# Ascend-Research/HeadPoseEstimation-WHENet

Hardware: NVIDIA H100
Metric: head-crops/sec @224x224 bf16 (higher is better)
Workload: dtype bf16

## Files before the change

headposeestimation-whenet_b200/csrc/kernels_fused.cuh:

```cuda
#pragma once
#include <algorithm>

#include "kernels_tc.cuh"

namespace whenet {
namespace fused {

using tc::BK;
using tc::BM;

constexpr size_t K1_MAX_SMEM = 227 * 1024 - 256;
constexpr float kDwScale = 4.0f;

struct K1Params {
    const void* in;
    const void* wt_aug;
    const float* w_dw;
    const void* w_dw16;
    const float* b_dw;
    void* out;
    float* partial;
    const float *w_se1t, *b_se1, *w_se2, *b_se2;
    float* gate;
    int* se_counter;
// ... 15 lines not shown
    int nkb;
    int pitchE;
    int PY;
    int spr_log2;
    int smem_A, smem_W, smem_C, smem_E;
    int* tflag;
    int chunks_per_cta;
};

__device__ __forceinline__ void cp_async16(uint32_t dst, const void* src, bool valid) {
    const uint32_t sz = valid ? 16u : 0u;
    asm volatile("cp.async.cg.shared.global [%0], [%1], 16, %2;" ::"r"(dst), "l"(src), "r"(sz) : "memory");
}
__device__ __forceinline__ void sts128(uint32_t addr, const uint4& v) {
    asm volatile("st.shared.v4.b32 [%0], {%1,%2,%3,%4};" ::"r"(addr), "r"(v.x), "r"(v.y), "r"(v.z), "r"(v.w) : "memory");
}
__device__ __forceinline__ void lds64(uint32_t addr, uint32_t& a, uint32_t& b) {
    asm volatile("ld.shared.v2.b32 {%0,%1}, [%2];" : "=r"(a), "=r"(b) : "r"(addr));
}
__device__ __forceinline__ float4 lds_f4(uint32_t addr) {
    float4 v;
    asm volatile("ld.shared.v4.f32 {%0,%1,%2,%3}, [%4];" : "=f"(v.x), "=f"(v.y), "=f"(v.z), "=f"(v.w) : "r"(addr));
    return v;
}
__device__ __forceinline__ void ffma2(float2& d, const float2& a, const float2& b) {
    d.x = fmaf(a.x, b.x, d.x);
    d.y = fmaf(a.y, b.y, d.y);
}
template <typename T> __device__ __forceinline__ void unpack2(uint32_t u, float& lo, float& hi);
template <> __device__ __forceinline__ void unpack2<__nv_bfloat16>(uint32_t u, float& lo, float& hi) {
    lo = __uint_as_float(u << 16);
    hi = __uint_as_float(u & 0xffff0000u);
}
template <> __device__ __forceinline__ void unpack2<__half>(uint32_t u, float& lo, float& hi) {
    const float2 f = __half22float2(*reinterpret_cast<const __half2*>(&u));
    lo = f.x; hi = f.y;
}
template <typename T> __device__ __forceinline__ uint32_t pack2(float lo, float hi);
template <> __device__ __forceinline__ uint32_t pack2<__nv_bfloat16>(float lo, float hi) {
    const __nv_bfloat162 h = __floats2bfloat162_rn(lo, hi);
    return *reinterpret_cast<const uint32_t*>(&h);
}
template <> __device__ __forceinline__ uint32_t pack2<__half>(float lo, float hi) {
    const __half2 h = __floats2half2_rn(lo, hi);
    return *reinterpret_cast<const uint32_t*>(&h);
}
template <typename T> __device__ __forceinline__ uint32_t ones2();
template <> __device__ __forceinline__ uint32_t ones2<__nv_bfloat16>() { return 0x3f803f80u; }
template <> __device__ __forceinline__ uint32_t ones2<__half>() { return 0x3c003c00u; }

__device__ __forceinline__ uint32_t sw128(int r, int c) {
    return (uint32_t)((r >> 3) * 1024 + (r & 7) * 128 + ((c ^ (r & 7)) << 4));
}

__device__ __forceinline__ int div_small(int x, float inv) { return __float2int_rz(((float)x + 0.5f) * inv); }

template <int NP>
__device__ __forceinline__ void expand_row_to_e(const float (&d)[8 * NP], int nch16, int hr, uint32_t er, int cq) {
#pragma unroll
    for (int jj = 0; jj < NP; ++jj) {
        if (jj < nch16) {
#pragma unroll
            for (int i = 0; i < 2; ++i) {
                const uint32_t v = pack2<__half>(swish_from_half(d[8 * jj + 4 * i + 2 * hr]), swish_from_half(d[8 * jj + 4 * i + 2 * hr + 1]));
                asm volatile("st.shared.b32 [%0], %1;" ::"r"(er + (uint32_t)(16 * jj + 8 * i + cq) * 2u), "r"(v) : "memory");
            }
        }
    }
}

template <int KS, int S, int R>
__device__ __forceinline__ void dw_strip_hfma2(uint32_t erow, uint32_t e_rowstride, uint32_t pitchE, uint32_t wts, uint32_t w_pitch,
                                               const float4& bq, float2 (&acc)[R][2]) {
    constexpr int NCOL = (R - 1) * S + KS;
    __half2 hacc[R][2];
#pragma unroll
    for (int r = 0; r < R; ++r) { hacc[r][0] = __float2half2_rn(0.f); hacc[r][1] = __float2half2_rn(0.f); }
#pragma unroll
    for (int ky = 0; ky < KS; ++ky) {
        __half2 wr[KS][2];
#pragma unroll
        for (int kx = 0; kx < KS; ++kx) {
            uint32_t w0, w1;
            lds64(wts + (uint32_t)(ky * KS + kx) * w_pitch, w0, w1);
            wr[kx][0] = *reinterpret_cast<__half2*>(&w0); wr[kx][1] = *reinterpret_cast<__half2*>(&w1);
        }
        uint32_t ea = erow;
#pragma unroll
        for (int col = 0; col < NCOL; ++col) {
            uint32_t a, b;
            lds64(ea, a, b);
            ea += pitchE;
            const __half2 x01 = *reinterpret_cast<__half2*>(&a), x23 = *reinterpret_cast<__half2*>(&b);
#pragma unroll
            for (int r = 0; r < R; ++r) {
                const int kx = col - r * S;
                if (kx >= 0 && kx < KS) {
                    hacc[r][0] = __hfma2(x01, wr[kx][0], hacc[r][0]);
                    hacc[r][1] = __hfma2(x23, wr[kx][1], hacc[r][1]);
                }
            }
        }
        erow += e_rowstride;
    }
    const float2 sc = make_float2(kDwScale, kDwScale);
#pragma unroll
// ... 480 lines not shown
```

headposeestimation-whenet_b200/csrc/kernels_k1x.cuh:

```cuda
#pragma once
#include "kernels_dwse.cuh"

namespace whenet {
namespace fused {

template <int KS, int S, int HIN, int TH, int R, int CC, int CIN>
struct K1X {
    static constexpr int NT = 256;
    static constexpr int HO = (HIN + S - 1) / S;
    static constexpr int PAD = ((HO - 1) * S + KS - HIN > 0 ? (HO - 1) * S + KS - HIN : 0) / 2;
    static constexpr int TILES_X = HO / TH, TILES = TILES_X * TILES_X;
    static constexpr int IW = (TH - 1) * S + KS;
    static constexpr int NPIX = IW * IW;
    static constexpr int HALVES = (NPIX + 63) / 64;
    static constexpr int KCH = CIN / 8;
    static constexpr int KSTEPS = ((KCH + 2) & ~1) >> 1;
    static constexpr int SPR = (TH + R - 1) / R;
    static constexpr int NSTRIPS = TH * SPR;
    static constexpr int CV = CC / 4;
    static constexpr int PY = NT / CV;
    static constexpr uint32_t PITCHE = CC * 2 + 16;
    static constexpr int E_ROWS = NPIX + R * S + 16;
    static_assert(HO % TH == 0 && CIN % 8 == 0 && KCH + 1 < 8 && CC % 16 == 0 && CC <= 128, "tile plan");
    static constexpr uint32_t A_BYTES = (NPIX + 7) / 8 * 8 * 128;
    static constexpr uint32_t A_TX = NPIX * 128;
    static constexpr uint32_t W_BYTES = CC * 128;
    static constexpr uint32_t E_BYTES = (E_ROWS * PITCHE + 127) / 128 * 128;
    static constexpr uint32_t DWW_BYTES = KS * KS * CC * 2;
    static constexpr uint32_t CST_TX = DWW_BYTES + CC * 4;
    static constexpr uint32_t CST_BYTES = (CST_TX + 127) / 128 * 128;
    static constexpr uint32_t RED_BYTES = PY * CC * 4;
    static constexpr uint32_t OFF_W = A_BYTES, OFF_E = OFF_W + 2 * W_BYTES, OFF_C = OFF_E + E_BYTES, OFF_R = OFF_C + 2 * CST_BYTES;
    static constexpr size_t SMEM = (size_t)OFF_R + 2 * RED_BYTES + 1024;
    static_assert((A_BYTES | W_BYTES) % 1024 == 0 && DWW_BYTES % 16 == 0, "operand alignment");
    static_assert((size_t)HALVES * 64 * 128 + 1024 <= SMEM, "the last half's MMA stays inside the CTA's window");
    static_assert(2 * (SMEM + 1024 + 64) <= 228 * 1024, "two CTAs per SM");
};

template <int KS, int S, int HIN, int TH, int R, int CC, int CIN>
__global__ void __launch_bounds__(256, 2) k1x_kernel(const __grid_constant__ DwSeParams p) {
    using X = K1X<KS, S, HIN, TH, R, CC, CIN>;
    using T = __nv_bfloat16;
    extern __shared__ uint8_t smem_k1x[];
    __shared__ __align__(8) uint64_t bars[5];
    __shared__ int s_abort_mem;
    volatile int* s_abort = &s_abort_mem;
    const uint32_t s0 = (tc::smem_u32(smem_k1x) + 1023u) & ~1023u;
    const uint32_t sA = s0, sW = s0 + X::OFF_W, sE = s0 + X::OFF_E, sC = s0 + X::OFF_C, sR = s0 + X::OFF_R;
    const uint32_t b_a = tc::smem_u32(&bars[0]), b_w = b_a + 8, b_c = b_a + 24;

    const int tid = threadIdx.x, warp = tid >> 5, lane = tid & 31;
    const int wg = tid >> 7, wq = warp & 3;
    const int tile = blockIdx.x, n = blockIdx.y;
    const int tyi = tile / X::TILES_X;
    const int ty0 = tyi * TH, tx0 = (tile - tyi * X::TILES_X) * TH;
    const int iy0 = ty0 * S - X::PAD, ix0 = tx0 * S - X::PAD;
    const int C = p.C, n_chunks = p.n_chunks;

    if (tid == 0) {
        for (int i = 0; i < 5; ++i) tc::mbar_init(&bars[i], 1);
        s_abort_mem = 0;
        asm volatile("fence.mbarrier_init.release.cluster;" ::: "memory");
        asm volatile("prefetch.tensormap [%0];" ::"l"(&p.tmX) : "memory");
        asm volatile("prefetch.tensormap [%0];" ::"l"(&p.tmWx) : "memory");
        asm volatile("prefetch.tensormap [%0];" ::"l"(&p.tmW) : "memory");
    }
    __syncthreads();

    auto issue_w = [&](int j) {
        const uint32_t bar = b_w + 8 * (j & 1);
        tc::mbar::arrive_expect_tx(bar, X::W_BYTES);
        tc::mbar::tma_2d(sW + (j & 1) * X::W_BYTES, &p.tmWx, 0, j * CC, bar);
    };
    auto issue_c = [&](int j) {
        const uint32_t bar = b_c + 8 * (j & 1), dst = sC + (j & 1) * X::CST_BYTES;
        tc::mbar::arrive_expect_tx(bar, X::CST_TX);
        tc::mbar::tma_2d(dst, &p.tmW, j * CC, 0, bar);
        asm volatile("cp.async.bulk.shared::cluster.global.mbarrier::complete_tx::bytes [%0], [%1], %2, [%3];"
                     ::"r"(dst + X::DWW_BYTES), "l"(p.b_dw + j * CC), "r"((uint32_t)(CC * 4)), "r"(bar) : "memory");
    };
    if (tid == 0) {
        tc::mbar::arrive_expect_tx(b_a, X::A_TX);
        tc::mbar::tma_4d(sA, &p.tmX, 0, ix0, iy0, n, b_a);
        issue_w(0); issue_c(0);
        if (n_chunks > 1) { issue_w(1); issue_c(1); }
    }

    const int py = tid / X::CV, cv = tid - py * X::CV;
    const bool dw_active = py < X::PY;
    T* const out_t = reinterpret_cast<T*>(p.out) + (((long long)n * X::HO + ty0) * X::HO + tx0) * C + cv * 4;

    tc::mbar::wait(b_a, 0, s_abort, p.tflag);
    for (int r = tid; r < X::NPIX; r += X::NT) {
        const int ty = r / X::IW, tx = r - ty * X::IW;
        const int iy = iy0 + ty, ix = ix0 + tx;
        if (iy >= 0 && iy < HIN && ix >= 0 && ix < HIN) sts128(sA + sw128(r, X::KCH), make_uint4(ones2<T>(), 0u, 0u, 0u));
    }
    asm volatile("fence.proxy.async.shared::cta;" ::: "memory");
    __syncthreads();

    for (int j = 0; j < n_chunks; ++j) {
        const int buf = j & 1;
        const uint32_t par = (uint32_t)(j >> 1) & 1u;
        tc::mbar::wait(b_w + 8 * buf, par, s_abort, p.tflag);
        for (int u = wg; u < X::HALVES; u += 2) {
            float d[CC / 2];
            tc::wg_mma_m64<true, CC>(d, sA + (uint32_t)u * 64 * 128, X::A_BYTES, sW + buf * X::W_BYTES, X::W_BYTES, X::KSTEPS);
            tc::wg_wait<0>();
            const int r_lo = u * 64 + 16 * wq + (lane >> 2), cq = 2 * (lane & 3);
#pragma unroll
            for (int hr = 0; hr < 2; ++hr) {
                const int r = r_lo + 8 * hr;
                if (r < X::NPIX) expand_row_to_e<CC / 16>(d, CC / 16, hr, sE + (uint32_t)r * X::PITCHE, cq);
            }
        }
        __syncthreads();
        if (tid == 0 && j + 2 < n_chunks) issue_w(j + 2);

        tc::mbar::wait(b_c + 8 * buf, par, s_abort, p.tflag);
        if (dw_active && !*s_abort) {
            const uint32_t cst = sC + buf * X::CST_BYTES;
            const float4 bq = lds_f4(cst + X::DWW_BYTES + (uint32_t)cv * 16);
            float sum[4] = {0.f, 0.f, 0.f, 0.f};
            for (int sidx = py; sidx < X::NSTRIPS; sidx += X::PY) {
                const int oyl = sidx / X::SPR, oxl0 = (sidx - oyl * X::SPR) * R;
                float2 acc[R][2];
                dw_strip_hfma2<KS, S, R>(sE + (uint32_t)((oyl * S * X::IW + oxl0 * S) * X::PITCHE + cv * 8), X::IW * X::PITCHE, X::PITCHE,
                                         cst + (uint32_t)cv * 8, CC * 2, bq, acc);
                dw_strip_finish<T, R>(acc, TH - oxl0, out_t + ((long long)oyl * X::HO + oxl0) * C + j * CC, C, sum);
            }
            asm volatile("st.shared.v4.f32 [%0], {%1,%2,%3,%4};" ::"r"(sR + (uint32_t)(buf * X::RED_BYTES + (py * CC + cv * 4) * 4)),
                         "f"(sum[0]), "f"(sum[1]), "f"(sum[2]), "f"(sum[3]) : "memory");
        }
        __syncthreads();
        if (warp == X::NT / 32 - 1) {
            squeeze_sums<X::PY, CC>(sR + buf * X::RED_BYTES, p.partial + ((long long)n * X::TILES + tile) * C + j * CC, nullptr, 0.f, lane);
            if (lane == 0 && j + 2 < n_chunks) issue_c(j + 2);
        }
    }
}

#define WHENET_K1X_INSTANCES(F) F(3, 2, 112, 8, 4, 48, 16) F(3, 1, 56, 14, 7, 48, 24) F(5, 2, 56, 7, 4, 48, 24) F(3, 2, 28, 7, 7, 80, 40)

inline bool k1x_has_instance(int k, int s, int hin, int cin, int pad, const K1Params& pl, int R) {
#define K1X_MATCH(KS_, S_, HIN_, TH_, R_, CC_, CIN_)                                                                        \
    if (k == KS_ && s == S_ && hin == HIN_ && cin == CIN_ && pl.TH == TH_ && pl.TW == TH_ && R == R_ && pl.CC == CC_ && pl.NB == 1 && \
        pad == K1X<KS_, S_, HIN_, TH_, R_, CC_, CIN_>::PAD)                                                                  \
        return true;
    WHENET_K1X_INSTANCES(K1X_MATCH)
#undef K1X_MATCH
    return false;
}

template <typename T>
int launch_k1x(cudaStream_t stream, DwSeParams p, int k, int s, int hin, int cin, int th, int r, int cc, int n_crops) {
    static_assert(std::is_same<T, __nv_bfloat16>::value, "K1X runs the bf16 wgmma and the HFMA2 depthwise");
    p.N = n_crops;
    p.n_chunks = p.C / cc;
    p.chunks_per_cta = p.n_chunks;
#define K1X_GO(KS, S, HIN, TH, RR, CC, CIN)                                                                                  \
    if (k == KS && s == S && hin == HIN && cin == CIN && th == TH && r == RR && cc == CC) {                                  \
        using X = K1X<KS, S, HIN, TH, RR, CC, CIN>;                                                                          \
        auto kfn = k1x_kernel<KS, S, HIN, TH, RR, CC, CIN>;                                                                  \
        if (cudaFuncSetAttribute(kfn, cudaFuncAttributeMaxDynamicSharedMemorySize, (int)X::SMEM) != cudaSuccess) return -1;  \
        kfn<<<dim3(X::TILES, n_crops), X::NT, X::SMEM, stream>>>(p);                                                         \
        return 0;                                                                                                            \
    }
    WHENET_K1X_INSTANCES(K1X_GO)
#undef K1X_GO
    return 1;
}

}
}
```

headposeestimation-whenet_b200/csrc/kernels_tc.cuh:

```cuda
#pragma once
#include <cuda.h>
#include <cuda_bf16.h>
#include <cuda_fp16.h>
#include <cuda_runtime.h>
#include <stdint.h>

#include "kernels_simt.cuh"

namespace whenet {
namespace tc {


constexpr int BM = 128;
constexpr int BK = 64;
constexpr int A_STAGE_BYTES = BM * BK * 2;
constexpr int kAccPitch = 132;
__host__ __device__ constexpr uint32_t acc_tile_bytes(int cols) { return (uint32_t)cols * kAccPitch * 4u; }

__device__ __forceinline__ uint32_t smem_u32(const void* p) { return (uint32_t)__cvta_generic_to_shared(p); }

__device__ __forceinline__ void mbar_init(uint64_t* bar, uint32_t count) {
    asm volatile("mbarrier.init.shared::cta.b64 [%0], %1;" ::"r"(smem_u32(bar)), "r"(count) : "memory");
}
__device__ __forceinline__ bool mbar_wait(uint64_t* bar, uint32_t parity, int* tflag) {
// ... 13 lines not shown

namespace mbar {

__device__ __forceinline__ void wait(uint32_t bar_addr, uint32_t parity, volatile int* abort_flag, int* tflag) {
    for (uint32_t outer = 0; outer < (1u << 18); ++outer) {
        uint32_t done;
        asm volatile(
            "{\n\t.reg .pred p;\n\t.reg .u32 n;\n\t"
            "mov.u32 n, 64;\n"
            "MBAR_POLL_%=:\n\t"
            "mbarrier.try_wait.parity.shared::cta.b64 p, [%1], %2;\n\t"
            "@p bra MBAR_DONE_%=;\n\t"
            "sub.u32 n, n, 1;\n\t"
            "setp.ne.u32 p, n, 0;\n\t"
            "@p bra MBAR_POLL_%=;\n\t"
            "setp.eq.u32 p, n, 1;\n"
            "MBAR_DONE_%=:\n\t"
            "selp.u32 %0, 1, 0, p;\n\t}"
            : "=r"(done) : "r"(bar_addr), "r"(parity) : "memory");
        if (done) return;
        if (*abort_flag) return;
    }
    *abort_flag = 1;
    *reinterpret_cast<volatile int*>(tflag) = 1;
}
__device__ __forceinline__ void arrive(uint32_t bar_addr) {
    asm volatile("mbarrier.arrive.shared::cta.b64 _, [%0];" ::"r"(bar_addr) : "memory");
}
__device__ __forceinline__ void arrive_warp(uint32_t bar_addr) {
    __syncwarp();
    if ((threadIdx.x & 31) == 0) arrive(bar_addr);
}
__device__ __forceinline__ void arrive_expect_tx(uint32_t bar_addr, uint32_t bytes) {
    asm volatile("mbarrier.arrive.expect_tx.shared::cta.b64 _, [%0], %1;" ::"r"(bar_addr), "r"(bytes) : "memory");
}
__device__ __forceinline__ void tma_4d(uint32_t dst, const CUtensorMap* tm, int c0, int c1, int c2, int c3, uint32_t bar_addr) {
    asm volatile("cp.async.bulk.tensor.4d.shared::cluster.global.mbarrier::complete_tx::bytes [%0], [%1, {%2, %3, %4, %5}], [%6];"
                 ::"r"(dst), "l"(tm), "r"(c0), "r"(c1), "r"(c2), "r"(c3), "r"(bar_addr) : "memory");
}
__device__ __forceinline__ void tma_2d(uint32_t dst, const CUtensorMap* tm, int c0, int c1, uint32_t bar_addr) {
    asm volatile("cp.async.bulk.tensor.2d.shared::cluster.global.mbarrier::complete_tx::bytes [%0], [%1, {%2, %3}], [%4];"
                 ::"r"(dst), "l"(tm), "r"(c0), "r"(c1), "r"(bar_addr) : "memory");
}

}

__device__ __forceinline__ uint64_t make_desc(uint32_t saddr) {
    uint64_t d = 0;
    d |= (uint64_t)((saddr >> 4) & 0x3FFF);
    d |= (uint64_t)1 << 16;
    d |= (uint64_t)64 << 32;
    d |= (uint64_t)1 << 62;
    return d;
}

__device__ __forceinline__ void wg_fence() { asm volatile("wgmma.fence.sync.aligned;" ::: "memory"); }
__device__ __forceinline__ void wg_commit() { asm volatile("wgmma.commit_group.sync.aligned;" ::: "memory"); }
template <int N> __device__ __forceinline__ void wg_wait() { asm volatile("wgmma.wait_group.sync.aligned %0;" ::"n"(N) : "memory"); }

#define WG_D8(g) "+f"(d[8 * g]), "+f"(d[8 * g + 1]), "+f"(d[8 * g + 2]), "+f"(d[8 * g + 3]), \
                 "+f"(d[8 * g + 4]), "+f"(d[8 * g + 5]), "+f"(d[8 * g + 6]), "+f"(d[8 * g + 7])
#define WG_OPS_1 WG_D8(0)
#define WG_OPS_2 WG_OPS_1, WG_D8(1)
#define WG_OPS_3 WG_OPS_2, WG_D8(2)
#define WG_OPS_4 WG_OPS_3, WG_D8(3)
#define WG_OPS_5 WG_OPS_4, WG_D8(4)
#define WG_OPS_6 WG_OPS_5, WG_D8(5)
#define WG_OPS_7 WG_OPS_6, WG_D8(6)
#define WG_OPS_8 WG_OPS_7, WG_D8(7)
#define WG_REGS_1 "%0,%1,%2,%3,%4,%5,%6,%7"
#define WG_REGS_2 WG_REGS_1 ",%8,%9,%10,%11,%12,%13,%14,%15"
#define WG_REGS_3 WG_REGS_2 ",%16,%17,%18,%19,%20,%21,%22,%23"
#define WG_REGS_4 WG_REGS_3 ",%24,%25,%26,%27,%28,%29,%30,%31"
#define WG_REGS_5 WG_REGS_4 ",%32,%33,%34,%35,%36,%37,%38,%39"
#define WG_REGS_6 WG_REGS_5 ",%40,%41,%42,%43,%44,%45,%46,%47"
#define WG_REGS_7 WG_REGS_6 ",%48,%49,%50,%51,%52,%53,%54,%55"
#define WG_REGS_8 WG_REGS_7 ",%56,%57,%58,%59,%60,%61,%62,%63"
#define WG_TAIL_1 "16", "%8, %9", "%10"
#define WG_TAIL_2 "32", "%16, %17", "%18"
#define WG_TAIL_3 "48", "%24, %25", "%26"
#define WG_TAIL_4 "64", "%32, %33", "%34"
#define WG_TAIL_5 "80", "%40, %41", "%42"
#define WG_TAIL_6 "96", "%48, %49", "%50"
#define WG_TAIL_7 "112", "%56, %57", "%58"
#define WG_TAIL_8 "128", "%64, %65", "%66"
#define WG_ASM_(TY, REGS, NS, AB, SC, ...)                                                                              \
    asm volatile("{\n\t.reg .pred p;\n\tsetp.ne.b32 p, " SC ", 0;\n\t"                                                    \
                 "wgmma.mma_async.sync.aligned.m64n" NS "k16.f32." TY "." TY " {" REGS "}, " AB ", p, 1, 1, 0, 0;\n\t}" \
                 : __VA_ARGS__ : "l"(ad), "l"(bd), "r"(accumulate))
#define WG_ASM(TY, REGS, TAIL, OPS) WG_ASM_(TY, REGS, TAIL, OPS)
#define WG_CASE(k)                                                                                                 \
    if constexpr (N == 16 * k) {                                                                                   \
        if constexpr (BF16) WG_ASM("bf16", WG_REGS_##k, WG_TAIL_##k, WG_OPS_##k);                                  \
        else WG_ASM("f16", WG_REGS_##k, WG_TAIL_##k, WG_OPS_##k);                                                  \
    }

template <bool BF16, int N>
__device__ __forceinline__ void wgmma(float (&d)[N / 2], uint64_t ad, uint64_t bd, uint32_t accumulate) {
    static_assert(N % 16 == 0 && N >= 16 && N <= 128, "wgmma: N = 16, 32, ..., 128");
    WG_CASE(1) WG_CASE(2) WG_CASE(3) WG_CASE(4) WG_CASE(5) WG_CASE(6) WG_CASE(7) WG_CASE(8)
}
#undef WG_CASE
#undef WG_ASM
#undef WG_ASM_

template <int N> struct WgAcc { float d[2][N / 2]; };
// ... 574 lines not shown
```

headposeestimation-whenet_b200/csrc/whenet_api.cu:

```cuda
#include <cuda_bf16.h>
#include <cuda_fp16.h>
#include <cuda_runtime.h>

#include <algorithm>
#include <atomic>
#include <cmath>
#include <cstdarg>
#include <cstdio>
#include <cstdlib>
#include <cstring>
#include <map>
#include <string>
#include <thread>
#include <type_traits>
#include <vector>

#include "../../include/whenet_b200.h"
#include "api_error.h"
#include "kernels_simt.cuh"
#include "kernels_tc.cuh"
#include "kernels_fused.cuh"
#include "kernels_crop.cuh"
#include "kernels_overlay.cuh"
#include "kernels_k2.cuh"
// ... 266 lines not shown
        if (*p) cudaFree(*p);
        *p = nullptr;
    }
    for (float** p : {&c->d_partial, &c->d_gate, &c->d_pooled}) {
        if (*p) cudaFree(*p);
        *p = nullptr;
    }
    if (c->d_se_counter) cudaFree(c->d_se_counter);
    c->d_se_counter = nullptr;
    c->ws_chunk = 0;
}

int ensure_ws(whenet_ctx* c) {
    if (c->ws_chunk == c->chunk && c->bufA) return 0;
    free_ws(c);
    const size_t es = esize(c->precision), ch = (size_t)c->chunk;
    size_t io = 112ull * 112 * 32, ex = 49ull * 1280, dw = 0, part = 0;
    for (const BlockCfg& b : c->blocks) {
        io = std::max(io, (size_t)b.hout * b.hout * b.cout);
        if (b.has_expand) ex = std::max(ex, (size_t)b.hin * b.hin * b.cexp);
        dw = std::max(dw, (size_t)b.hout * b.hout * b.cexp);
        part = std::max(part, (size_t)((b.hout + 7) / 8) * b.cexp);
    }
    for (const K1Plan& pl : c->k1)
        if (pl.valid) part = std::max(part, (size_t)pl.p.tiles_x * pl.p.tiles_y * pl.p.Cexp);
    const BlockCfg& b1 = c->blocks[0];
    if (c->precision == WHENET_PRECISION_BF16) part = std::max(part, (size_t)(b1.hin / 14) * (b1.hin / 14) * b1.cexp);
    if (c->dw1.valid) part = std::max(part, (size_t)c->dw1.p.tiles_x * c->dw1.p.tiles_y * c->dw1.p.Cexp);
    c->ws_io = io; c->ws_ex = ex; c->ws_dw = dw; c->ws_part = part;
    CK(cudaMalloc(&c->bufA, ch * io * es));
    CK(cudaMalloc(&c->bufB, ch * io * es));
    CK(cudaMalloc(&c->bufE, ch * ex * es));
    CK(cudaMalloc(&c->bufD, ch * dw * es));
    CK(cudaMalloc(&c->d_partial, ch * part * sizeof(float)));
    CK(cudaMalloc(&c->d_gate, ch * 1152 * sizeof(float)));
    CK(cudaMalloc(&c->d_pooled, ch * 1280 * sizeof(float)));
    CK(cudaMalloc(&c->d_se_counter, ch * sizeof(int)));
    CK(cudaMemset(c->d_se_counter, 0, ch * sizeof(int)));
    for (int i = 0; i < 2; ++i) CK(cudaMalloc(&c->d_in[i], ch * kImgElems * sizeof(float)));
    c->ws_chunk = c->chunk;
    return 0;
}

PFN_cuTensorMapEncodeTiled_v12000 tmap_encode_fn() {
    static PFN_cuTensorMapEncodeTiled_v12000 fn = nullptr;
    if (!fn) {
        void* f = nullptr;
        cudaDriverEntryPointQueryResult q;
        if (cudaGetDriverEntryPoint("cuTensorMapEncodeTiled", &f, cudaEnableDefault, &q) == cudaSuccess && q == cudaDriverEntryPointSuccess)
            fn = reinterpret_cast<PFN_cuTensorMapEncodeTiled_v12000>(f);
    }
    return fn;
}
int make_tmap_w(CUtensorMap* tm, const void* base, int rows, int K, int box_rows, bool is_bf16) {
    auto fn = tmap_encode_fn();
    if (!fn) return fail(WHENET_ECUDA, "cuTensorMapEncodeTiled is not available from this driver");
    const cuuint64_t dims[2] = {(cuuint64_t)K, (cuuint64_t)rows};
    const cuuint64_t strides[1] = {(cuuint64_t)K * 2};
    const cuuint32_t box[2] = {64, (cuuint32_t)box_rows};
    const cuuint32_t estr[2] = {1, 1};
    const CUresult r = fn(tm, is_bf16 ? CU_TENSOR_MAP_DATA_TYPE_BFLOAT16 : CU_TENSOR_MAP_DATA_TYPE_FLOAT16, 2, const_cast<void*>(base), dims, strides,
                          box, estr, CU_TENSOR_MAP_INTERLEAVE_NONE, CU_TENSOR_MAP_SWIZZLE_128B, CU_TENSOR_MAP_L2_PROMOTION_L2_256B,
                          CU_TENSOR_MAP_FLOAT_OOB_FILL_NONE);
    if (r != CUDA_SUCCESS) return fail(WHENET_ECUDA, "cuTensorMapEncodeTiled(weights %dx%d, box %d) failed: %d", rows, K, box_rows, (int)r);
    return 0;
}

int make_tmap_kd_e(CUtensorMap* tm, const void* base, int n, int H, int C, int cc, int pw) {
    auto fn = tmap_encode_fn();
    if (!fn) return fail(WHENET_ECUDA, "cuTensorMapEncodeTiled is not available from this driver");
    const cuuint64_t dims[4] = {(cuuint64_t)C, (cuuint64_t)H, (cuuint64_t)H, (cuuint64_t)n};
    const cuuint64_t strides[3] = {(cuuint64_t)C * 2, (cuuint64_t)H * C * 2, (cuuint64_t)H * H * C * 2};
    const cuuint32_t box[4] = {(cuuint32_t)cc, (cuuint32_t)pw, (cuuint32_t)pw, 1};
    const cuuint32_t estr[4] = {1, 1, 1, 1};
    const CUresult r = fn(tm, CU_TENSOR_MAP_DATA_TYPE_FLOAT16, 4, const_cast<void*>(base), dims, strides, box, estr, CU_TENSOR_MAP_INTERLEAVE_NONE,
                          CU_TENSOR_MAP_SWIZZLE_NONE, CU_TENSOR_MAP_L2_PROMOTION_L2_128B, CU_TENSOR_MAP_FLOAT_OOB_FILL_NONE);
    if (r != CUDA_SUCCESS) return fail(WHENET_ECUDA, "cuTensorMapEncodeTiled(KD tile %dx%dx%dx%d, box %dx%dx%d) failed: %d", n, H, H, C, pw, pw, cc, (int)r);
    return 0;
}
int make_tmap_k1x_in(CUtensorMap* tm, const void* base, int n, int H, int C, int iw) {
    auto fn = tmap_encode_fn();
    if (!fn) return fail(WHENET_ECUDA, "cuTensorMapEncodeTiled is not available from this driver");
    const cuuint64_t dims[4] = {(cuuint64_t)C, (cuuint64_t)H, (cuuint64_t)H, (cuuint64_t)n};
    const cuuint64_t strides[3] = {(cuuint64_t)C * 2, (cuuint64_t)H * C * 2, (cuuint64_t)H * H * C * 2};
    const cuuint32_t box[4] = {64, (cuuint32_t)iw, (cuuint32_t)iw, 1};
    const cuuint32_t estr[4] = {1, 1, 1, 1};
    const CUresult r = fn(tm, CU_TENSOR_MAP_DATA_TYPE_BFLOAT16, 4, const_cast<void*>(base), dims, strides, box, estr, CU_TENSOR_MAP_INTERLEAVE_NONE,
                          CU_TENSOR_MAP_SWIZZLE_128B, CU_TENSOR_MAP_L2_PROMOTION_L2_128B, CU_TENSOR_MAP_FLOAT_OOB_FILL_NONE);
    if (r != CUDA_SUCCESS) return fail(WHENET_ECUDA, "cuTensorMapEncodeTiled(K1X input %dx%dx%dx%d, box %dx%d) failed: %d", n, H, H, C, iw, iw, (int)r);
    return 0;
}
int make_tmap_kd_w(CUtensorMap* tm, const void* base, int kk, int C, int cc) {
    auto fn = tmap_encode_fn();
    if (!fn) return fail(WHENET_ECUDA, "cuTensorMapEncodeTiled is not available from this driver");
    const cuuint64_t dims[2] = {(cuuint64_t)C, (cuuint64_t)kk};
    const cuuint64_t strides[1] = {(cuuint64_t)C * 2};
    const cuuint32_t box[2] = {(cuuint32_t)cc, (cuuint32_t)kk};
    const cuuint32_t estr[2] = {1, 1};
    const CUresult r = fn(tm, CU_TENSOR_MAP_DATA_TYPE_FLOAT16, 2, const_cast<void*>(base), dims, strides, box, estr, CU_TENSOR_MAP_INTERLEAVE_NONE,
                          CU_TENSOR_MAP_SWIZZLE_NONE, CU_TENSOR_MAP_L2_PROMOTION_L2_128B, CU_TENSOR_MAP_FLOAT_OOB_FILL_NONE);
    if (r != CUDA_SUCCESS) return fail(WHENET_ECUDA, "cuTensorMapEncodeTiled(KD weights %dx%d, box %d) failed: %d", kk, C, cc, (int)r);
    return 0;
}

template <typename T>
int launch_pw(whenet_ctx* c, const char* name, const T* A, const float* W, const void* Wt16, const float* bias,
              const float* gate, const T* resid, T* out, long long M, int K, int N, int hw, bool swish, bool out_half = false) {
    const double bytes = (double)M * (K + N + (resid ? N : 0)) * sizeof(T);
    const double flops = 2.0 * (double)M * K * N;
    Scope sc(c, name, bytes, flops);
    if constexpr (sizeof(T) == 2) {
        const bool want_k2 = c->pw_variant == 3 || (c->pw_variant == 4 && (gate == nullptr || hw <= 196));
        if (c->use_tc && Wt16 && want_k2 && !out_half) {
            whenet::tc::K2Params kp{};
            size_t smem = 0;
            if (whenet::tc::plan_k2(M, K, N, hw, gate != nullptr, c->precision == WHENET_PRECISION_BF16, &kp, &smem) &&
                (c->pw_variant == 3 || kp.tiles >= 2 * c->sm_count)) {
                if (c->tmaps2.size() > 1024) c->tmaps2.clear();
                const TmapKey ka{K, (int)M, (const void*)A}, kw{-N, K, Wt16};
                auto ia = c->tmaps2.find(ka);
                if (ia == c->tmaps2.end()) {
                    CUtensorMap tm;
                    int rc = make_tmap_w(&tm, A, (int)M, K, whenet::tc::BM, c->precision == WHENET_PRECISION_BF16);
                    if (rc) return rc;
                    ia = c->tmaps2.emplace(ka, tm).first;
                }
                auto iw = c->tmaps2.find(kw);
                if (iw == c->tmaps2.end()) {
                    CUtensorMap tm;
                    int rc = make_tmap_w(&tm, Wt16, N, K, kp.n_tile, c->precision == WHENET_PRECISION_BF16);
                    if (rc) return rc;
                    iw = c->tmaps2.emplace(kw, tm).first;
                }
                kp.tmA = ia->second; kp.tmW = iw->second;
                kp.bias = bias; kp.gate = gate; kp.resid = resid; kp.out = out; kp.tflag = c->d_tflag;
                int rc = whenet::tc::launch_k2<T>(c->stream, kp, smem, swish, gate != nullptr, resid != nullptr, c->sm_count);
                if (rc == 0) { CK(cudaGetLastError()); return 0; }
                if (rc < 0) return fail(WHENET_ECUDA, "K2 launch failed for %s (rc=%d)", name, rc);
            }
        }
        if (c->use_tc && Wt16 && gate && hw >= 784 && c->pw3 && !out_half && !swish) {
// ... 203 lines not shown
                p.w_se1t = w.w_se1t; p.b_se1 = w.b_se1; p.w_se2 = w.w_se2; p.b_se2 = w.b_se2; p.gate = c->d_gate; p.Cse = b.cse;
                p.inv_hw = 1.0f / (float)(b.hout * b.hout);
                p.C = b.cexp; p.pad = b.pad;
                if (split == 1 && c->se_tail && c->kd_tail) {
                    p.se_tail = 1;
                    se_in_k1 = true;
                    if (c->se_scale_out && !taps) { p.scale_out = 1; d_gated = true; }
                }
                snprintf(nm, sizeof nm, "b%02d.kd", b.idx);
                if (split == 1) {
                    Scope sc(c, nm, (double)nb * ((double)b.hin * b.hin * b.cin + (double)b.hout * b.hout * b.cexp) * sizeof(T),
                             2.0 * nb * ((double)b.hin * b.hin * b.cin * b.cexp + (double)b.hout * b.hout * b.k * b.k * b.cexp));
                    rc = whenet::fused::launch_dwse_x<T>(c->stream, p, b.k, b.s, b.hin, b.cin, nb);
                    if (rc != 0) return fail(WHENET_ECUDA, "KD (on-chip expand) launch failed for block %d (rc=%d)", b.idx, rc);
                    CK(cudaGetLastError());
                } else {
                    Scope sc(c, nm, (double)nb * ((double)b.hin * b.hin + (double)b.hout * b.hout) * b.cexp * sizeof(T),
                             2.0 * nb * (double)b.hout * b.hout * b.k * b.k * b.cexp);
                    rc = whenet::fused::launch_dwse<T>(c->stream, p, b.k, b.s, b.hin, nb, split);
                    if (rc != 0) return fail(WHENET_ECUDA, "KD launch failed for block %d (rc=%d)", b.idx, rc);
                    CK(cudaGetLastError());
                }
                tiles = 1;
                did_k1 = true;
              }
            } else if (c->use_fused && c->k1[i].valid && b.idx <= c->fused_max_block) {
                whenet::fused::K1Params p = c->k1[i].p;
                p.in = cur; p.wt_aug = w.wt_exp_aug; p.w_dw = w.w_dw_h; p.w_dw16 = w.w_dw16; p.b_dw = w.b_dw_h; p.out = D; p.partial = c->d_partial; p.tflag = c->d_tflag;
                p.w_se1t = w.w_se1t; p.b_se1 = w.b_se1; p.w_se2 = w.w_se2; p.b_se2 = w.b_se2; p.gate = c->d_gate; p.Cse = b.cse;
                se_in_k1 = c->se_fused && p.NB == 1;
                p.se_counter = se_in_k1 ? c->d_se_counter : nullptr;
                {
                    const long long ctas = (long long)p.tiles_x * p.tiles_y * ((nb + p.NB - 1) / p.NB);
                    int split = 1;
                    while (split < p.n_chunks && ctas * split < c->k1_split_ctas) ++split;
                    p.chunks_per_cta = (p.n_chunks + split - 1) / split;
                    if (c->se_tail && !se_in_k1 && p.tiles_x * p.tiles_y == 1 && split == 1) {
                        p.se_tail = 1;
                        p.inv_hw = 1.0f / (float)(b.hout * b.hout);
                        se_in_k1 = true;
                        if (c->se_scale_out && !taps) { p.scale_out = 1; d_gated = true; }
                    }
                }
                snprintf(nm, sizeof nm, "b%02d.k1", b.idx);
                Scope sc(c, nm, (double)nb * ((double)b.hin * b.hin * b.cin + (double)b.hout * b.hout * b.cexp) * sizeof(T),
                         2.0 * nb * ((double)b.hin * b.hin * b.cin * b.cexp + (double)b.hout * b.hout * b.k * b.k * b.cexp));
                bool did_k1x = false;
                if constexpr (std::is_same<T, __nv_bfloat16>::value) {
                    if (c->k1x && c->use_tc && p.chunks_per_cta == p.n_chunks && !se_in_k1 &&
                        whenet::fused::k1x_has_instance(b.k, b.s, b.hin, b.cin, b.pad, p, c->k1[i].R)) {
                        whenet::fused::DwSeParams q{};
                        int rc = 0;
                        if (c->tmaps.size() > 512) c->tmaps.clear();
                        const TmapKey kx{600 + b.idx, nb, (const void*)cur}, kwx{700 + b.idx, 0, (const void*)w.wt_exp_aug}, kw{500 + b.idx, 0, (const void*)w.w_dw16};
                        auto ix = c->tmaps.find(kx);
                        if (ix == c->tmaps.end()) {
                            CUtensorMap tm;
                            if ((rc = make_tmap_k1x_in(&tm, cur, nb, b.hin, b.cin, p.IW))) return rc;
                            ix = c->tmaps.emplace(kx, tm).first;
                        }
                        auto iwx = c->tmaps.find(kwx);
                        if (iwx == c->tmaps.end()) {
                            CUtensorMap tm;
                            if ((rc = make_tmap_w(&tm, w.wt_exp_aug, b.cexp, b.cin + 8, p.CC, true))) return rc;
                            iwx = c->tmaps.emplace(kwx, tm).first;
                        }
                        auto iw = c->tmaps.find(kw);
                        if (iw == c->tmaps.end()) {
                            CUtensorMap tm;
                            if ((rc = make_tmap_kd_w(&tm, w.w_dw16, b.k * b.k, b.cexp, p.CC))) return rc;
                            iw = c->tmaps.emplace(kw, tm).first;
                        }
                        q.tmX = ix->second; q.tmWx = iwx->second; q.tmW = iw->second;
                        q.b_dw = w.b_dw_h; q.tflag = c->d_tflag; q.out = D; q.partial = c->d_partial; q.C = b.cexp; q.pad = b.pad;
                        rc = whenet::fused::launch_k1x<T>(c->stream, q, b.k, b.s, b.hin, b.cin, p.TH, c->k1[i].R, p.CC, nb);
                        if (rc != 0) return fail(WHENET_ECUDA, "K1X launch failed for block %d (rc=%d)", b.idx, rc);
                        CK(cudaGetLastError());
                        did_k1x = true;
                    }
                }
                if (!did_k1x) {
                    int rc = whenet::fused::launch_k1<T>(c->stream, p, b.k, b.s, c->k1[i].R, c->k1[i].NT, c->k1[i].smem, nb);
                    if (rc != 0) return fail(WHENET_ECUDA, "K1 launch failed for block %d (rc=%d)", b.idx, rc);
                    CK(cudaGetLastError());
                }
                tiles = p.tiles_x * p.tiles_y;
                did_k1 = true;
            }
        }
        if (!did_k1) {
        if (b.has_expand) {
            snprintf(nm, sizeof nm, "b%02d.expand", b.idx);
            int rc = launch_pw<T>(c, nm, cur, w.w_exp, w.wt_exp, w.b_exp, nullptr, nullptr, E,
                                  (long long)nb * b.hin * b.hin, b.cin, b.cexp, b.hin * b.hin, true);
            if (rc) return rc;
            dw_in = E;
        }
        snprintf(nm, sizeof nm, "b%02d.dw", b.idx);
        int rc = launch_dw<T>(c, nm, b, w, dw_in, D, nb, &tiles);
        if (rc) return rc;
        }
        int rc = 0;
        if (!se_in_k1) {
            snprintf(nm, sizeof nm, "b%02d.se", b.idx);
            Scope sc(c, nm, (double)nb * (tiles + 1) * b.cexp * 4.0, 4.0 * nb * b.cexp * b.cse);
            const float inv_hw = 1.0f / (float)(b.hout * b.hout);
            const size_t se_smem = (b.cexp + b.cse) * sizeof(float);
            if (nb >= 64 && c->se_batch) {
                constexpr int SEB = 4;
                whenet::se_gate_batch_kernel<SEB, 512><<<(nb + SEB - 1) / SEB, 512, SEB * se_smem, c->stream>>>(
                    c->d_partial, tiles, inv_hw, w.w_se1t, w.b_se1, w.w_se2, w.b_se2, c->d_gate, b.cexp, b.cse, nb);
            } else if (nb < 64 || c->se_wide)
                whenet::se_gate_kernel<1024><<<nb, 1024, se_smem, c->stream>>>(
                    c->d_partial, tiles, inv_hw, w.w_se1t, w.b_se1, w.w_se2, w.b_se2, c->d_gate, b.cexp, b.cse);
            else
                whenet::se_gate_kernel<256><<<nb, 256, se_smem, c->stream>>>(
                    c->d_partial, tiles, inv_hw, w.w_se1t, w.b_se1, w.w_se2, w.b_se2, c->d_gate, b.cexp, b.cse);
// ... 1268 lines not shown
```

Baseline: 80140.

## Use 64B-swizzled operand rows and a persistent tile loop in K1X

For blocks with small input channel counts (cin+8 <= 32), the K1X kernel now stores the A and weight operands in 64-byte swizzled rows instead of 128-byte rows. This halves their shared-memory footprint and allows three CTAs per SM instead of two. The kernel also becomes persistent: the grid is capped at occupancy times SM count, and each CTA loops over (crop, tile) items. The next tile's input TMA is prefetched during the last chunk, and the weight double-buffers run continuously across items. This adds descriptor and swizzle variants plus a device-attribute query at every launch, and risks stale weight-buffer parity or wrong phase tracking when prefetching across items.

```diff
diff --git a/headposeestimation-whenet_b200/csrc/kernels_fused.cuh b/headposeestimation-whenet_b200/csrc/kernels_fused.cuh
--- a/headposeestimation-whenet_b200/csrc/kernels_fused.cuh
+++ b/headposeestimation-whenet_b200/csrc/kernels_fused.cuh
@@ -91,6 +91,9 @@
 __device__ __forceinline__ uint32_t sw128(int r, int c) {
     return (uint32_t)((r >> 3) * 1024 + (r & 7) * 128 + ((c ^ (r & 7)) << 4));
 }
+__device__ __forceinline__ uint32_t sw64(int r, int c) {
+    return (uint32_t)(r * 64 + ((c ^ ((r >> 1) & 3)) << 4));
+}
 
 __device__ __forceinline__ int div_small(int x, float inv) { return __float2int_rz(((float)x + 0.5f) * inv); }
 
diff --git a/headposeestimation-whenet_b200/csrc/kernels_k1x.cuh b/headposeestimation-whenet_b200/csrc/kernels_k1x.cuh
--- a/headposeestimation-whenet_b200/csrc/kernels_k1x.cuh
+++ b/headposeestimation-whenet_b200/csrc/kernels_k1x.cuh
@@ -3,6 +3,8 @@
 
 namespace whenet {
 namespace fused {
+
+__host__ __device__ constexpr int k1x_row_bytes(int cin) { return cin + 8 <= 32 ? 64 : 128; }
 
 template <int KS, int S, int HIN, int TH, int R, int CC, int CIN>
 struct K1X {
@@ -15,16 +17,19 @@
     static constexpr int HALVES = (NPIX + 63) / 64;
     static constexpr int KCH = CIN / 8;
     static constexpr int KSTEPS = ((KCH + 2) & ~1) >> 1;
+    static constexpr int ROWB = k1x_row_bytes(CIN);
+    static constexpr uint32_t ATOM = 8 * ROWB;
+    static constexpr int CTAS_PER_SM = ROWB == 64 ? 3 : 2;
     static constexpr int SPR = (TH + R - 1) / R;
     static constexpr int NSTRIPS = TH * SPR;
     static constexpr int CV = CC / 4;
     static constexpr int PY = NT / CV;
     static constexpr uint32_t PITCHE = CC * 2 + 16;
     static constexpr int E_ROWS = NPIX + R * S + 16;
-    static_assert(HO % TH == 0 && CIN % 8 == 0 && KCH + 1 < 8 && CC % 16 == 0 && CC <= 128, "tile plan");
-    static constexpr uint32_t A_BYTES = (NPIX + 7) / 8 * 8 * 128;
-    static constexpr uint32_t A_TX = NPIX * 128;
-    static constexpr uint32_t W_BYTES = CC * 128;
+    static_assert(HO % TH == 0 && CIN % 8 == 0 && KSTEPS * 32 <= ROWB && CC % 16 == 0 && CC <= 128, "tile plan");
+    static constexpr uint32_t A_BYTES = (NPIX + 7) / 8 * ATOM;
+    static constexpr uint32_t A_TX = NPIX * ROWB;
+    static constexpr uint32_t W_BYTES = CC * ROWB;
     static constexpr uint32_t E_BYTES = (E_ROWS * PITCHE + 127) / 128 * 128;
     static constexpr uint32_t DWW_BYTES = KS * KS * CC * 2;
     static constexpr uint32_t CST_TX = DWW_BYTES + CC * 4;
@@ -32,13 +37,14 @@
     static constexpr uint32_t RED_BYTES = PY * CC * 4;
     static constexpr uint32_t OFF_W = A_BYTES, OFF_E = OFF_W + 2 * W_BYTES, OFF_C = OFF_E + E_BYTES, OFF_R = OFF_C + 2 * CST_BYTES;
     static constexpr size_t SMEM = (size_t)OFF_R + 2 * RED_BYTES + 1024;
-    static_assert((A_BYTES | W_BYTES) % 1024 == 0 && DWW_BYTES % 16 == 0, "operand alignment");
-    static_assert((size_t)HALVES * 64 * 128 + 1024 <= SMEM, "the last half's MMA stays inside the CTA's window");
-    static_assert(2 * (SMEM + 1024 + 64) <= 228 * 1024, "two CTAs per SM");
+    static_assert((A_BYTES | W_BYTES) % ATOM == 0 && OFF_E % 128 == 0 && DWW_BYTES % 16 == 0, "operand alignment");
+    static_assert((size_t)HALVES * 64 * ROWB + 1024 <= SMEM, "the last half's MMA stays inside the CTA's window");
+    static_assert(CTAS_PER_SM * (SMEM + 1024 + 256) <= 228 * 1024, "CTAS_PER_SM CTAs per SM");
+    __device__ static uint32_t sw(int r, int c) { return ROWB == 64 ? sw64(r, c) : sw128(r, c); }
 };
 
 template <int KS, int S, int HIN, int TH, int R, int CC, int CIN>
-__global__ void __launch_bounds__(256, 2) k1x_kernel(const __grid_constant__ DwSeParams p) {
+__global__ void __launch_bounds__(256, (K1X<KS, S, HIN, TH, R, CC, CIN>::CTAS_PER_SM)) k1x_kernel(const __grid_constant__ DwSeParams p) {
     using X = K1X<KS, S, HIN, TH, R, CC, CIN>;
     using T = __nv_bfloat16;
     extern __shared__ uint8_t smem_k1x[];
@@ -51,11 +57,10 @@
 
     const int tid = threadIdx.x, warp = tid >> 5, lane = tid & 31;
     const int wg = tid >> 7, wq = warp & 3;
-    const int tile = blockIdx.x, n = blockIdx.y;
-    const int tyi = tile / X::TILES_X;
-    const int ty0 = tyi * TH, tx0 = (tile - tyi * X::TILES_X) * TH;
-    const int iy0 = ty0 * S - X::PAD, ix0 = tx0 * S - X::PAD;
     const int C = p.C, n_chunks = p.n_chunks;
+    const int items = p.N * X::TILES;
+    const int n_items = (items - (int)blockIdx.x + (int)gridDim.x - 1) / (int)gridDim.x;
+    const int n_g = n_items * n_chunks;
 
     if (tid == 0) {
         for (int i = 0; i < 5; ++i) tc::mbar_init(&bars[i], 1);
@@ -67,75 +72,91 @@
     }
     __syncthreads();
 
-    auto issue_w = [&](int j) {
-        const uint32_t bar = b_w + 8 * (j & 1);
+    auto issue_a = [&](int item) {
+        const int n = item / X::TILES, tile = item - n * X::TILES, tyi = tile / X::TILES_X;
+        tc::mbar::arrive_expect_tx(b_a, X::A_TX);
+        tc::mbar::tma_4d(sA, &p.tmX, 0, (tile - tyi * X::TILES_X) * TH * S - X::PAD, tyi * TH * S - X::PAD, n, b_a);
+    };
+    auto issue_w = [&](int g, int j) {
+        const uint32_t bar = b_w + 8 * (g & 1);
         tc::mbar::arrive_expect_tx(bar, X::W_BYTES);
-        tc::mbar::tma_2d(sW + (j & 1) * X::W_BYTES, &p.tmWx, 0, j * CC, bar);
+        tc::mbar::tma_2d(sW + (g & 1) * X::W_BYTES, &p.tmWx, 0, j * CC, bar);
     };
-    auto issue_c = [&](int j) {
-        const uint32_t bar = b_c + 8 * (j & 1), dst = sC + (j & 1) * X::CST_BYTES;
+    auto issue_c = [&](int g, int j) {
+        const uint32_t bar = b_c + 8 * (g & 1), dst = sC + (g & 1) * X::CST_BYTES;
         tc::mbar::arrive_expect_tx(bar, X::CST_TX);
         tc::mbar::tma_2d(dst, &p.tmW, j * CC, 0, bar);
         asm volatile("cp.async.bulk.shared::cluster.global.mbarrier::complete_tx::bytes [%0], [%1], %2, [%3];"
                      ::"r"(dst + X::DWW_BYTES), "l"(p.b_dw + j * CC), "r"((uint32_t)(CC * 4)), "r"(bar) : "memory");
     };
     if (tid == 0) {
-        tc::mbar::arrive_expect_tx(b_a, X::A_TX);
-        tc::mbar::tma_4d(sA, &p.tmX, 0, ix0, iy0, n, b_a);
-        issue_w(0); issue_c(0);
-        if (n_chunks > 1) { issue_w(1); issue_c(1); }
+        issue_a(blockIdx.x);
+        issue_w(0, 0); issue_c(0, 0);
+        if (n_g > 1) { issue_w(1, 1 % n_chunks); issue_c(1, 1 % n_chunks); }
     }
 
     const int py = tid / X::CV, cv = tid - py * X::CV;
     const bool dw_active = py < X::PY;
-    T* const out_t = reinterpret_cast<T*>(p.out) + (((long long)n * X::HO + ty0) * X::HO + tx0) * C + cv * 4;
-
-    tc::mbar::wait(b_a, 0, s_abort, p.tflag);
-    for (int r = tid; r < X::NPIX; r += X::NT) {
-        const int ty = r / X::IW, tx = r - ty * X::IW;
-        const int iy = iy0 + ty, ix = ix0 + tx;
-        if (iy >= 0 && iy < HIN && ix >= 0 && ix < HIN) sts128(sA + sw128(r, X::KCH), make_uint4(ones2<T>(), 0u, 0u, 0u));
-    }
-    asm volatile("fence.proxy.async.shared::cta;" ::: "memory");
-    __syncthreads();
-
-    for (int j = 0; j < n_chunks; ++j) {
-        const int buf = j & 1;
-        const uint32_t par = (uint32_t)(j >> 1) & 1u;
-        tc::mbar::wait(b_w + 8 * buf, par, s_abort, p.tflag);
-        for (int u = wg; u < X::HALVES; u += 2) {
-            float d[CC / 2];
-            tc::wg_mma_m64<true, CC>(d, sA + (uint32_t)u * 64 * 128, X::A_BYTES, sW + buf * X::W_BYTES, X::W_BYTES, X::KSTEPS);
-            tc::wg_wait<0>();
-            const int r_lo = u * 64 + 16 * wq + (lane >> 2), cq = 2 * (lane & 3);
+
+    int g = 0;
+    for (int k = 0, item = blockIdx.x; k < n_items; ++k, item += gridDim.x) {
+        const int n = item / X::TILES, tile = item - n * X::TILES;
+        const int tyi = tile / X::TILES_X;
+        const int ty0 = tyi * TH, tx0 = (tile - tyi * X::TILES_X) * TH;
+        const int iy0 = ty0 * S - X::PAD, ix0 = tx0 * S - X::PAD;
+        T* const out_t = reinterpret_cast<T*>(p.out) + (((long long)n * X::HO + ty0) * X::HO + tx0) * C + cv * 4;
+
+        tc::mbar::wait(b_a, (uint32_t)k & 1u, s_abort, p.tflag);
+        for (int r = tid; r < X::NPIX; r += X::NT) {
+            const int ty = r / X::IW, tx = r - ty * X::IW;
+            const int iy = iy0 + ty, ix = ix0 + tx;
+            if (iy >= 0 && iy < HIN && ix >= 0 && ix < HIN) sts128(sA + X::sw(r, X::KCH), make_uint4(ones2<T>(), 0u, 0u, 0u));
+        }
+        asm volatile("fence.proxy.async.shared::cta;" ::: "memory");
+        if (__syncthreads_or(*s_abort)) return;
+
+        for (int j = 0; j < n_chunks; ++j, ++g) {
+            const int buf = g & 1;
+            const uint32_t par = (uint32_t)(g >> 1) & 1u;
+            tc::mbar::wait(b_w + 8 * buf, par, s_abort, p.tflag);
+            for (int u = wg; u < X::HALVES; u += 2) {
+                float d[CC / 2];
+                tc::wg_mma_block<true, CC, 1>(*reinterpret_cast<float(*)[1][CC / 2]>(&d), tc::make_desc_rows<X::ROWB>(sA + (uint32_t)u * 64 * X::ROWB), 0,
+                                              tc::make_desc_rows<X::ROWB>(sW + buf * X::W_BYTES), X::KSTEPS, 0u);
+                tc::wg_wait<0>();
+                const int r_lo = u * 64 + 16 * wq + (lane >> 2), cq = 2 * (lane & 3);
 #pragma unroll
-            for (int hr = 0; hr < 2; ++hr) {
-                const int r = r_lo + 8 * hr;
-                if (r < X::NPIX) expand_row_to_e<CC / 16>(d, CC / 16, hr, sE + (uint32_t)r * X::PITCHE, cq);
-            }
-        }
-        __syncthreads();
-        if (tid == 0 && j + 2 < n_chunks) issue_w(j + 2);
-
-        tc::mbar::wait(b_c + 8 * buf, par, s_abort, p.tflag);
-        if (dw_active && !*s_abort) {
-            const uint32_t cst = sC + buf * X::CST_BYTES;
-            const float4 bq = lds_f4(cst + X::DWW_BYTES + (uint32_t)cv * 16);
-            float sum[4] = {0.f, 0.f, 0.f, 0.f};
-            for (int sidx = py; sidx < X::NSTRIPS; sidx += X::PY) {
-                const int oyl = sidx / X::SPR, oxl0 = (sidx - oyl * X::SPR) * R;
-                float2 acc[R][2];
-                dw_strip_hfma2<KS, S, R>(sE + (uint32_t)((oyl * S * X::IW + oxl0 * S) * X::PITCHE + cv * 8), X::IW * X::PITCHE, X::PITCHE,
-                                         cst + (uint32_t)cv * 8, CC * 2, bq, acc);
-                dw_strip_finish<T, R>(acc, TH - oxl0, out_t + ((long long)oyl * X::HO + oxl0) * C + j * CC, C, sum);
-            }
-            asm volatile("st.shared.v4.f32 [%0], {%1,%2,%3,%4};" ::"r"(sR + (uint32_t)(buf * X::RED_BYTES + (py * CC + cv * 4) * 4)),
-                         "f"(sum[0]), "f"(sum[1]), "f"(sum[2]), "f"(sum[3]) : "memory");
-        }
-        __syncthreads();
-        if (warp == X::NT / 32 - 1) {
-            squeeze_sums<X::PY, CC>(sR + buf * X::RED_BYTES, p.partial + ((long long)n * X::TILES + tile) * C + j * CC, nullptr, 0.f, lane);
-            if (lane == 0 && j + 2 < n_chunks) issue_c(j + 2);
+                for (int hr = 0; hr < 2; ++hr) {
+                    const int r = r_lo + 8 * hr;
+                    if (r < X::NPIX) expand_row_to_e<CC / 16>(d, CC / 16, hr, sE + (uint32_t)r * X::PITCHE, cq);
+                }
+            }
+            __syncthreads();
+            if (tid == 0) {
+                if (j == n_chunks - 1 && k + 1 < n_items) issue_a(item + gridDim.x);
+                if (g + 2 < n_g) issue_w(g + 2, (j + 2) % n_chunks);
+            }
+
+            tc::mbar::wait(b_c + 8 * buf, par, s_abort, p.tflag);
+            if (dw_active && !*s_abort) {
+                const uint32_t cst = sC + buf * X::CST_BYTES;
+                const float4 bq = lds_f4(cst + X::DWW_BYTES + (uint32_t)cv * 16);
+                float sum[4] = {0.f, 0.f, 0.f, 0.f};
+                for (int sidx = py; sidx < X::NSTRIPS; sidx += X::PY) {
+                    const int oyl = sidx / X::SPR, oxl0 = (sidx - oyl * X::SPR) * R;
+                    float2 acc[R][2];
+                    dw_strip_hfma2<KS, S, R>(sE + (uint32_t)((oyl * S * X::IW + oxl0 * S) * X::PITCHE + cv * 8), X::IW * X::PITCHE, X::PITCHE,
+                                             cst + (uint32_t)cv * 8, CC * 2, bq, acc);
+                    dw_strip_finish<T, R>(acc, TH - oxl0, out_t + ((long long)oyl * X::HO + oxl0) * C + j * CC, C, sum);
+                }
+                asm volatile("st.shared.v4.f32 [%0], {%1,%2,%3,%4};" ::"r"(sR + (uint32_t)(buf * X::RED_BYTES + (py * CC + cv * 4) * 4)),
+                             "f"(sum[0]), "f"(sum[1]), "f"(sum[2]), "f"(sum[3]) : "memory");
+            }
+            __syncthreads();
+            if (warp == X::NT / 32 - 1) {
+                squeeze_sums<X::PY, CC>(sR + buf * X::RED_BYTES, p.partial + ((long long)n * X::TILES + tile) * C + j * CC, nullptr, 0.f, lane);
+                if (lane == 0 && g + 2 < n_g) issue_c(g + 2, (j + 2) % n_chunks);
+            }
         }
     }
 }
@@ -163,7 +184,12 @@
         using X = K1X<KS, S, HIN, TH, RR, CC, CIN>;                                                                          \
         auto kfn = k1x_kernel<KS, S, HIN, TH, RR, CC, CIN>;                                                                  \
         if (cudaFuncSetAttribute(kfn, cudaFuncAttributeMaxDynamicSharedMemorySize, (int)X::SMEM) != cudaSuccess) return -1;  \
-        kfn<<<dim3(X::TILES, n_crops), X::NT, X::SMEM, stream>>>(p);                                                         \
+        int dev = 0, sms = 0, per_sm = 0;                                                                                    \
+        if (cudaGetDevice(&dev) != cudaSuccess || cudaDeviceGetAttribute(&sms, cudaDevAttrMultiProcessorCount, dev) != cudaSuccess || \
+            cudaOccupancyMaxActiveBlocksPerMultiprocessor(&per_sm, kfn, X::NT, X::SMEM) != cudaSuccess || per_sm < 1)        \
+            return -1;                                                                                                       \
+        const long long items = (long long)X::TILES * n_crops;                                                               \
+        kfn<<<(unsigned)std::min(items, (long long)per_sm * sms), X::NT, X::SMEM, stream>>>(p);                              \
         return 0;                                                                                                            \
     }
     WHENET_K1X_INSTANCES(K1X_GO)
diff --git a/headposeestimation-whenet_b200/csrc/kernels_tc.cuh b/headposeestimation-whenet_b200/csrc/kernels_tc.cuh
--- a/headposeestimation-whenet_b200/csrc/kernels_tc.cuh
+++ b/headposeestimation-whenet_b200/csrc/kernels_tc.cuh
@@ -89,6 +89,20 @@
     d |= (uint64_t)64 << 32;
     d |= (uint64_t)1 << 62;
     return d;
+}
+__device__ __forceinline__ uint64_t make_desc_sw64(uint32_t saddr) {
+    uint64_t d = 0;
+    d |= (uint64_t)((saddr >> 4) & 0x3FFF);
+    d |= (uint64_t)1 << 16;
+    d |= (uint64_t)32 << 32;
+    d |= (uint64_t)2 << 62;
+    return d;
+}
+template <int ROWB>
+__device__ __forceinline__ uint64_t make_desc_rows(uint32_t saddr) {
+    static_assert(ROWB == 64 || ROWB == 128, "rows of 64 or 128 bytes");
+    if constexpr (ROWB == 64) return make_desc_sw64(saddr);
+    else return make_desc(saddr);
 }
 
 __device__ __forceinline__ void wg_fence() { asm volatile("wgmma.fence.sync.aligned;" ::: "memory"); }
diff --git a/headposeestimation-whenet_b200/csrc/whenet_api.cu b/headposeestimation-whenet_b200/csrc/whenet_api.cu
--- a/headposeestimation-whenet_b200/csrc/whenet_api.cu
+++ b/headposeestimation-whenet_b200/csrc/whenet_api.cu
@@ -342,15 +342,16 @@
     }
     return fn;
 }
-int make_tmap_w(CUtensorMap* tm, const void* base, int rows, int K, int box_rows, bool is_bf16) {
+int make_tmap_w(CUtensorMap* tm, const void* base, int rows, int K, int box_rows, bool is_bf16, int row_bytes = 128) {
     auto fn = tmap_encode_fn();
     if (!fn) return fail(WHENET_ECUDA, "cuTensorMapEncodeTiled is not available from this driver");
     const cuuint64_t dims[2] = {(cuuint64_t)K, (cuuint64_t)rows};
     const cuuint64_t strides[1] = {(cuuint64_t)K * 2};
-    const cuuint32_t box[2] = {64, (cuuint32_t)box_rows};
+    const cuuint32_t box[2] = {(cuuint32_t)row_bytes / 2, (cuuint32_t)box_rows};
     const cuuint32_t estr[2] = {1, 1};
     const CUresult r = fn(tm, is_bf16 ? CU_TENSOR_MAP_DATA_TYPE_BFLOAT16 : CU_TENSOR_MAP_DATA_TYPE_FLOAT16, 2, const_cast<void*>(base), dims, strides,
-                          box, estr, CU_TENSOR_MAP_INTERLEAVE_NONE, CU_TENSOR_MAP_SWIZZLE_128B, CU_TENSOR_MAP_L2_PROMOTION_L2_256B,
+                          box, estr, CU_TENSOR_MAP_INTERLEAVE_NONE, row_bytes == 64 ? CU_TENSOR_MAP_SWIZZLE_64B : CU_TENSOR_MAP_SWIZZLE_128B,
+                          CU_TENSOR_MAP_L2_PROMOTION_L2_256B,
                           CU_TENSOR_MAP_FLOAT_OOB_FILL_NONE);
     if (r != CUDA_SUCCESS) return fail(WHENET_ECUDA, "cuTensorMapEncodeTiled(weights %dx%d, box %d) failed: %d", rows, K, box_rows, (int)r);
     return 0;
@@ -368,15 +369,16 @@
     if (r != CUDA_SUCCESS) return fail(WHENET_ECUDA, "cuTensorMapEncodeTiled(KD tile %dx%dx%dx%d, box %dx%dx%d) failed: %d", n, H, H, C, pw, pw, cc, (int)r);
     return 0;
 }
-int make_tmap_k1x_in(CUtensorMap* tm, const void* base, int n, int H, int C, int iw) {
+int make_tmap_k1x_in(CUtensorMap* tm, const void* base, int n, int H, int C, int iw, int row_bytes) {
     auto fn = tmap_encode_fn();
     if (!fn) return fail(WHENET_ECUDA, "cuTensorMapEncodeTiled is not available from this driver");
     const cuuint64_t dims[4] = {(cuuint64_t)C, (cuuint64_t)H, (cuuint64_t)H, (cuuint64_t)n};
     const cuuint64_t strides[3] = {(cuuint64_t)C * 2, (cuuint64_t)H * C * 2, (cuuint64_t)H * H * C * 2};
-    const cuuint32_t box[4] = {64, (cuuint32_t)iw, (cuuint32_t)iw, 1};
+    const cuuint32_t box[4] = {(cuuint32_t)row_bytes / 2, (cuuint32_t)iw, (cuuint32_t)iw, 1};
     const cuuint32_t estr[4] = {1, 1, 1, 1};
     const CUresult r = fn(tm, CU_TENSOR_MAP_DATA_TYPE_BFLOAT16, 4, const_cast<void*>(base), dims, strides, box, estr, CU_TENSOR_MAP_INTERLEAVE_NONE,
-                          CU_TENSOR_MAP_SWIZZLE_128B, CU_TENSOR_MAP_L2_PROMOTION_L2_128B, CU_TENSOR_MAP_FLOAT_OOB_FILL_NONE);
+                          row_bytes == 64 ? CU_TENSOR_MAP_SWIZZLE_64B : CU_TENSOR_MAP_SWIZZLE_128B, CU_TENSOR_MAP_L2_PROMOTION_L2_128B,
+                          CU_TENSOR_MAP_FLOAT_OOB_FILL_NONE);
     if (r != CUDA_SUCCESS) return fail(WHENET_ECUDA, "cuTensorMapEncodeTiled(K1X input %dx%dx%dx%d, box %dx%d) failed: %d", n, H, H, C, iw, iw, (int)r);
     return 0;
 }
@@ -686,17 +688,18 @@
                         whenet::fused::DwSeParams q{};
                         int rc = 0;
                         if (c->tmaps.size() > 512) c->tmaps.clear();
+                        const int rowb = whenet::fused::k1x_row_bytes(b.cin);
                         const TmapKey kx{600 + b.idx, nb, (const void*)cur}, kwx{700 + b.idx, 0, (const void*)w.wt_exp_aug}, kw{500 + b.idx, 0, (const void*)w.w_dw16};
                         auto ix = c->tmaps.find(kx);
                         if (ix == c->tmaps.end()) {
                             CUtensorMap tm;
-                            if ((rc = make_tmap_k1x_in(&tm, cur, nb, b.hin, b.cin, p.IW))) return rc;
+                            if ((rc = make_tmap_k1x_in(&tm, cur, nb, b.hin, b.cin, p.IW, rowb))) return rc;
                             ix = c->tmaps.emplace(kx, tm).first;
                         }
                         auto iwx = c->tmaps.find(kwx);
                         if (iwx == c->tmaps.end()) {
                             CUtensorMap tm;
-                            if ((rc = make_tmap_w(&tm, w.wt_exp_aug, b.cexp, b.cin + 8, p.CC, true))) return rc;
+                            if ((rc = make_tmap_w(&tm, w.wt_exp_aug, b.cexp, b.cin + 8, p.CC, true, rowb))) return rc;
                             iwx = c->tmaps.emplace(kwx, tm).first;
                         }
                         auto iw = c->tmaps.find(kw);
```

New measurement: 84690, median of 6. +5.7%, better.
